# bupt-cist/vqa-playground-pytorch

Measured on AMD Instinct MI355X. Metric: VQA samples/sec (fwd+bwd), CoR2 batch 512, 36x2048 regions, higher is better.
Workload: dtype f32

## Files before the change

### vqa_playground_pytorch_amd/csrc/bilinear_rt.hip

```cpp
#include <cstdlib>

#include "bilinear_folded.hpp"
#include "gemm_f32_rt.hpp"

namespace vqa {
namespace {

struct FoldRtArgs {
  const float* x;
  const float* w[2];
  const float* bias[2];
  const float* h2;
  float* out;
  int ldx, ldw, ldh2, ldo;
  int B, N, K, NO;
  int tiles_o;
};

constexpr int kNB = 3;

template <bool FWD, int S, int IB, int R, int FG = 1>
__global__ __launch_bounds__(rt::kThreads, 1) void bilinear_fold_rt_kernel(FoldRtArgs p) {
  using rt::f32x4;
  const int lane = threadIdx.x & 63, r = lane & 15, g = lane >> 4;
  const int wave = __builtin_amdgcn_readfirstlane(threadIdx.x >> 6);
  const int tile = xcd_remap(blockIdx.x, gridDim.x);
  const int b0 = (tile / p.tiles_o) * S;
  const int o0 = (tile % p.tiles_o) * (64 * IB) + wave * (16 * IB);
  const int B = p.B, N = p.N, K = p.K, NO = p.NO;
  if (o0 >= NO) return;

  rt::rsrc_t Wb[R];
#pragma unroll
  for (int rk = 0; rk < R; ++rk) Wb[rk] = rt::make_rsrc(p.w[rk], ((size_t)(NO - 1) * p.ldw + K) * 4);
  const rt::rsrc_t Xb = rt::make_rsrc(p.x, ((size_t)(B * N - 1) * p.ldx + K) * 4);
  const rt::rsrc_t Hb = rt::make_rsrc(p.h2, (size_t)B * R * p.ldh2 * 4);
  uint32_t offW[IB], offX[S][kNB], offH[S];
#pragma unroll
  for (int i = 0; i < IB; ++i) offW[i] = ((uint32_t)min(o0 + 16 * i + r, NO - 1) * (uint32_t)p.ldw + 4u * g) * 4u;
#pragma unroll
  for (int s = 0; s < S; ++s) {
    const int b = min(b0 + s, B - 1);
#pragma unroll
    for (int j = 0; j < kNB; ++j) offX[s][j] = ((uint32_t)(b * N + min(16 * j + r, N - 1)) * (uint32_t)p.ldx + 4u * g) * 4u;
    offH[s] = (uint32_t)(b * R) * (uint32_t)p.ldh2 * 4u;
  }
  float hrow[FWD ? S : 1][R][FWD ? IB : 1];
  if constexpr (FWD) {
#pragma unroll
    for (int s = 0; s < S; ++s)
#pragma unroll
      for (int rk = 0; rk < R; ++rk)
#pragma unroll
        for (int i = 0; i < IB; ++i)
          hrow[s][rk][i] = rt::ldg4(Hb, offH[s] + (uint32_t)(rk * p.ldh2 + min(o0 + 16 * i + r, NO - 1)) * 4u, 0u);
  }

  f32x4 acc[S][IB][kNB];
#pragma unroll
  for (int s = 0; s < S; ++s)
#pragma unroll
    for (int i = 0; i < IB; ++i)
#pragma unroll
      for (int j = 0; j < kNB; ++j) acc[s][i][j] = f32x4{0.f, 0.f, 0.f, 0.f};

  struct Frag {
    f32x4 w[R][IB];
    f32x4 x[S][kNB];
    f32x4 hk[FWD ? 1 : S][R];
  };
  auto load = [&](Frag& f, int c) {
    const uint32_t so = (uint32_t)c * 64u;
#pragma unroll
    for (int rk = 0; rk < R; ++rk)
#pragma unroll
      for (int i = 0; i < IB; ++i) f.w[rk][i] = rt::ldg16(Wb[rk], offW[i], so);
#pragma unroll
    for (int s = 0; s < S; ++s) {
#pragma unroll
      for (int j = 0; j < kNB; ++j) f.x[s][j] = rt::ldg16(Xb, offX[s][j], so);
      if constexpr (!FWD) {
#pragma unroll
        for (int rk = 0; rk < R; ++rk) f.hk[s][rk] = rt::ldg16(Hb, offH[s] + (uint32_t)(rk * p.ldh2) * 4u + 16u * g, so);
      }
    }
  };
  auto fold = [&](const Frag& f, int s, int i) -> f32x4 {
    typedef float f32x2 __attribute__((ext_vector_type(2)));
    f32x4 we;
    if constexpr (FWD) {
      const f32x2 h0 = f32x2{hrow[s][0][i], hrow[s][0][i]};
      f32x2 lo = f32x2{f.w[0][i][0], f.w[0][i][1]} * h0, hi = f32x2{f.w[0][i][2], f.w[0][i][3]} * h0;
      if constexpr (R == 2) {
        const f32x2 h1 = f32x2{hrow[s][1][i], hrow[s][1][i]};
        lo = __builtin_elementwise_fma(f32x2{f.w[1][i][0], f.w[1][i][1]}, h1, lo);
        hi = __builtin_elementwise_fma(f32x2{f.w[1][i][2], f.w[1][i][3]}, h1, hi);
      }
      we = f32x4{lo[0], lo[1], hi[0], hi[1]};
    } else {
      f32x2 lo = f32x2{f.w[0][i][0], f.w[0][i][1]} * f32x2{f.hk[s][0][0], f.hk[s][0][1]};
      f32x2 hi = f32x2{f.w[0][i][2], f.w[0][i][3]} * f32x2{f.hk[s][0][2], f.hk[s][0][3]};
      if constexpr (R == 2) {
        lo = __builtin_elementwise_fma(f32x2{f.w[1][i][0], f.w[1][i][1]}, f32x2{f.hk[s][1][0], f.hk[s][1][1]}, lo);
        hi = __builtin_elementwise_fma(f32x2{f.w[1][i][2], f.w[1][i][3]}, f32x2{f.hk[s][1][2], f.hk[s][1][3]}, hi);
      }
      we = f32x4{lo[0], lo[1], hi[0], hi[1]};
    }
    return we;
  };
  auto compute = [&](const Frag& f, auto pin, auto nloads) {
    constexpr bool PIN = decltype(pin)::value;
    constexpr int NL = decltype(nloads)::value;
    constexpr int NQ = S * IB;
    constexpr int NV = R == 2 ? 4 : 2;
    f32x4 we[FG], wn[FG];
#pragma unroll
    for (int t = 0; t < FG; ++t) we[t] = fold(f, min(t, NQ - 1) / IB, min(t, NQ - 1) % IB);
    if constexpr (PIN) __builtin_amdgcn_sched_group_barrier(0x002, NV * FG, 0);
    int issued = 0;
#pragma unroll
    for (int q0 = 0; q0 < NQ; q0 += FG) {
#pragma unroll
      for (int t = 0; t < FG; ++t) wn[t] = we[t];
      if (q0 + FG < NQ) {
#pragma unroll
        for (int t = 0; t < FG; ++t)
          if (q0 + FG + t < NQ) {
            wn[t] = fold(f, (q0 + FG + t) / IB, (q0 + FG + t) % IB);
            if constexpr (PIN) __builtin_amdgcn_sched_group_barrier(0x002, NV, 0);
          }
      }
#pragma unroll
      for (int t = 0; t < FG; ++t) {
        const int q = q0 + t;
        if (q >= NQ) break;
        const int s = q / IB, i = q % IB;
#pragma unroll
        for (int kb = 0; kb < 4; ++kb)
#pragma unroll
          for (int j = 0; j < kNB; ++j) {
            acc[s][i][j] = __builtin_amdgcn_mfma_f32_16x16x4f32(we[t][kb], f.x[s][j][kb], acc[s][i][j], 0, 0, 0);
            if constexpr (PIN) {
              __builtin_amdgcn_sched_group_barrier(0x008, 1, 0);
              const int m = q * 4 * kNB + kb * kNB + j;
              if (issued < NL && (m + 1) * NL / (NQ * 4 * kNB) > issued) {
                __builtin_amdgcn_sched_group_barrier(0x020, 1, 0);
                ++issued;
              }
            }
          }
      }
#pragma unroll
      for (int t = 0; t < FG; ++t) we[t] = wn[t];
    }
  };
  auto step = [&](Frag& fn, int cn, const Frag& f) {
    constexpr int NL = R * IB + S * kNB + (FWD ? 0 : S * R);
    load(fn, cn);
    compute(f, std::true_type{}, std::integral_constant<int, NL>{});
    __builtin_amdgcn_sched_barrier(0);
  };

  const int nfull = K >> 4;
  const int c_pairs = nfull & ~1;
  {
    Frag f0, f1;
    if (c_pairs > 0) {
      load(f0, 0);
      __builtin_amdgcn_sched_barrier(0);
      for (int c = 0; c < c_pairs; c += 2) {
        step(f1, c + 1, f0);
        step(f0, min(c + 2, c_pairs - 1), f1);
      }
    }
    if (c_pairs < nfull) {
      load(f0, c_pairs);
      compute(f0, std::false_type{}, std::integral_constant<int, 0>{});
    }
  }
  if ((K & 15) != 0 || FWD) {
    Frag f;
#pragma unroll
    for (int kb = 0; kb < 4; ++kb) {
      const int k = 16 * nfull + 4 * g + kb;
      const bool in = k < K;
      const uint32_t kc = (uint32_t)min(k, K - 1);
#pragma unroll
      for (int rk = 0; rk < R; ++rk)
#pragma unroll
        for (int i = 0; i < IB; ++i) {
          float v = rt::ldg4(Wb[rk], offW[i] - 16u * g + kc * 4u, 0u);
          v = in ? v : 0.f;
          if constexpr (FWD) {
            if (k == K) v = p.bias[rk][min(o0 + 16 * i + r, NO - 1)];
          }
          f.w[rk][i][kb] = v;
        }
#pragma unroll
      for (int s = 0; s < S; ++s) {
#pragma unroll
        for (int j = 0; j < kNB; ++j) {
          float v = rt::ldg4(Xb, offX[s][j] - 16u * g + kc * 4u, 0u);
          v = in ? v : 0.f;
          if constexpr (FWD) {
            if (k == K) v = 1.f;
          }
          f.x[s][j][kb] = v;
        }
        if constexpr (!FWD) {
#pragma unroll
          for (int rk = 0; rk < R; ++rk) {
            const float v = rt::ldg4(Hb, offH[s] + (uint32_t)(rk * p.ldh2) * 4u + kc * 4u, 0u);
            f.hk[s][rk][kb] = in ? v : 0.f;
          }
        }
      }
    }
    compute(f, std::false_type{}, std::integral_constant<int, 0>{});
  }

#pragma unroll
  for (int s = 0; s < S; ++s) {
    const int b = b0 + s;
    if (b >= B) break;
#pragma unroll
    for (int j = 0; j < kNB; ++j) {
      const int n = 16 * j + r;
      if (n >= N) continue;
      float* __restrict__ row = p.out + (size_t)(b * N + n) * p.ldo;
#pragma unroll
      for (int i = 0; i < IB; ++i) {
        const int o = o0 + 16 * i + 4 * g;
        if (o + 3 < NO) {
          *reinterpret_cast<f32x4*>(row + o) = acc[s][i][j];
        } else {
#pragma unroll
          for (int t = 0; t < 4; ++t)
            if (o + t < NO) row[o + t] = acc[s][i][j][t];
        }
      }
    }
  }
}

template <bool FWD>
int launch(const FoldRtArgs& a0, int R, hipStream_t s) {
  FoldRtArgs a = a0;
  constexpr int S = FWD ? 4 : 2, IB = FWD ? 4 : 5;
  a.tiles_o = (a.NO + 64 * IB - 1) / (64 * IB);
  const dim3 grid((unsigned)(((a.B + S - 1) / S) * a.tiles_o));
  const char* fg_opt = vqa::option("VQA_K4_FG");
  const int fg = fg_opt != nullptr ? std::atoi(fg_opt) : (FWD ? 4 : 2);
  if (R == 1)
    VQA_LAUNCH((bilinear_fold_rt_kernel<FWD, S, IB, 1>), grid, dim3(rt::kThreads), 0, s, a);
  else if (fg == 2)
    VQA_LAUNCH((bilinear_fold_rt_kernel<FWD, S, IB, 2, 2>), grid, dim3(rt::kThreads), 0, s, a);
  else if (fg == 4)
    VQA_LAUNCH((bilinear_fold_rt_kernel<FWD, S, IB, 2, 4>), grid, dim3(rt::kThreads), 0, s, a);
  else
    VQA_LAUNCH((bilinear_fold_rt_kernel<FWD, S, IB, 2>), grid, dim3(rt::kThreads), 0, s, a);
  return check_launch(FWD ? "lowrank_bilinear_fusion_folded_fwd (register-tile)" : "lowrank_bilinear_fusion_folded_bwd (dx, register-tile)");
}

}

bool fold_rt_supported(int B, int N, int K, int NO, int R, int ldx, int ldw, int ldo) {
  const bool off = vqa::option_is("VQA_K4_RT", '0');
  return !off && R >= 1 && R <= 2 && N > 16 && N <= 48 && B >= 256 && K >= 32 && NO >= 64 && ldx % 2 == 0 && ldw % 2 == 0 &&
         ldo % 2 == 0 && (size_t)B * N * (size_t)(ldx > ldo ? ldx : ldo) * 4 < (1ull << 32) && (size_t)NO * ldw * 4 < (1ull << 32);
}

int fold_rt_forward(const float* x, int ldx, const float* const* w1, const float* const* b1, const float* h2, float* out, int B,
                    int N, int L, int H, int R, hipStream_t s) {
  FoldRtArgs a{};
  a.x = x;
  for (int r = 0; r < R; ++r) {
    a.w[r] = w1[r];
    a.bias[r] = b1[r];
  }
  a.h2 = h2;
  a.out = out;
  a.ldx = ldx;
  a.ldw = L;
  a.ldh2 = H;
  a.ldo = H;
  a.B = B;
  a.N = N;
  a.K = L;
  a.NO = H;
  return launch<true>(a, R, s);
}

int fold_rt_data_gradient(const float* g, const float* const* w1t, const float* h2, float* d_x, int B, int N, int L, int H, int R,
                          hipStream_t s) {
  FoldRtArgs a{};
  a.x = g;
  for (int r = 0; r < R; ++r) a.w[r] = w1t[r];
  a.h2 = h2;
  a.out = d_x;
  a.ldx = H;
  a.ldw = H;
  a.ldh2 = H;
  a.ldo = L;
  a.B = B;
  a.N = N;
  a.K = H;
  a.NO = L;
  return launch<false>(a, R, s);
}

}
```

Baseline: 262,900.

## Pack leftover regions of four samples into one shared MFMA block in fold forward

```diff
diff --git a/vqa_playground_pytorch_amd/csrc/bilinear_rt.hip b/vqa_playground_pytorch_amd/csrc/bilinear_rt.hip
--- a/vqa_playground_pytorch_amd/csrc/bilinear_rt.hip
+++ b/vqa_playground_pytorch_amd/csrc/bilinear_rt.hip
@@ -17,11 +17,11 @@
   int tiles_o;
 };
 
-constexpr int kNB = 3;
-
-template <bool FWD, int S, int IB, int R, int FG = 1>
+template <bool FWD, int S, int IB, int R, int FG = 1, int NBF = 3, bool LEFT = false>
 __global__ __launch_bounds__(rt::kThreads, 1) void bilinear_fold_rt_kernel(FoldRtArgs p) {
   using rt::f32x4;
+  static_assert(!LEFT || (FWD && S == 4), "the shared leftover block is the forward's: 4 samples x 4 regions");
+  constexpr int kNB = NBF;
   const int lane = threadIdx.x & 63, r = lane & 15, g = lane >> 4;
   const int wave = __builtin_amdgcn_readfirstlane(threadIdx.x >> 6);
   const int tile = xcd_remap(blockIdx.x, gridDim.x);
@@ -45,6 +45,9 @@
     for (int j = 0; j < kNB; ++j) offX[s][j] = ((uint32_t)(b * N + min(16 * j + r, N - 1)) * (uint32_t)p.ldx + 4u * g) * 4u;
     offH[s] = (uint32_t)(b * R) * (uint32_t)p.ldh2 * 4u;
   }
+  uint32_t offXL = 0u;
+  if constexpr (LEFT)
+    offXL = ((uint32_t)(min(b0 + (r >> 2), B - 1) * N + min(16 * NBF + (r & 3), N - 1)) * (uint32_t)p.ldx + 4u * g) * 4u;
   float hrow[FWD ? S : 1][R][FWD ? IB : 1];
   if constexpr (FWD) {
 #pragma unroll
@@ -63,10 +66,16 @@
     for (int i = 0; i < IB; ++i)
 #pragma unroll
       for (int j = 0; j < kNB; ++j) acc[s][i][j] = f32x4{0.f, 0.f, 0.f, 0.f};
+  f32x4 accL[LEFT ? R : 1][LEFT ? IB : 1];
+#pragma unroll
+  for (int rk = 0; rk < (LEFT ? R : 1); ++rk)
+#pragma unroll
+    for (int i = 0; i < (LEFT ? IB : 1); ++i) accL[rk][i] = f32x4{0.f, 0.f, 0.f, 0.f};
 
   struct Frag {
     f32x4 w[R][IB];
     f32x4 x[S][kNB];
+    f32x4 xl;
     f32x4 hk[FWD ? 1 : S][R];
   };
   auto load = [&](Frag& f, int c) {
@@ -84,6 +93,7 @@
         for (int rk = 0; rk < R; ++rk) f.hk[s][rk] = rt::ldg16(Hb, offH[s] + (uint32_t)(rk * p.ldh2) * 4u + 16u * g, so);
       }
     }
+    if constexpr (LEFT) f.xl = rt::ldg16(Xb, offXL, so);
   };
   auto fold = [&](const Frag& f, int s, int i) -> f32x4 {
     typedef float f32x2 __attribute__((ext_vector_type(2)));
@@ -113,11 +123,15 @@
     constexpr int NL = decltype(nloads)::value;
     constexpr int NQ = S * IB;
     constexpr int NV = R == 2 ? 4 : 2;
+    constexpr int NG = (NQ + FG - 1) / FG;
+    constexpr int NML = LEFT ? 4 * R * IB : 0;
+    constexpr int NM = NQ * 4 * kNB + NML;
+    static_assert(NML % NG == 0, "the shared block's MFMAs divide evenly over the fold groups");
     f32x4 we[FG], wn[FG];
 #pragma unroll
     for (int t = 0; t < FG; ++t) we[t] = fold(f, min(t, NQ - 1) / IB, min(t, NQ - 1) % IB);
     if constexpr (PIN) __builtin_amdgcn_sched_group_barrier(0x002, NV * FG, 0);
-    int issued = 0;
+    int issued = 0, m = 0;
 #pragma unroll
     for (int q0 = 0; q0 < NQ; q0 += FG) {
 #pragma unroll
@@ -130,6 +144,22 @@
             if constexpr (PIN) __builtin_amdgcn_sched_group_barrier(0x002, NV, 0);
           }
       }
+      if constexpr (LEFT) {
+#pragma unroll
+        for (int u0 = 0; u0 < NML / NG; ++u0) {
+          const int u = (q0 / FG) * (NML / NG) + u0;
+          const int kb = u / (R * IB), rk = (u / IB) % R, i = u % IB;
+          accL[rk][i] = __builtin_amdgcn_mfma_f32_16x16x4f32(f.w[rk][i][kb], f.xl[kb], accL[rk][i], 0, 0, 0);
+          if constexpr (PIN) {
+            __builtin_amdgcn_sched_group_barrier(0x008, 1, 0);
+            if (issued < NL && (m + 1) * NL / NM > issued) {
+              __builtin_amdgcn_sched_group_barrier(0x020, 1, 0);
+              ++issued;
+            }
+          }
+          ++m;
+        }
+      }
 #pragma unroll
       for (int t = 0; t < FG; ++t) {
         const int q = q0 + t;
@@ -142,12 +172,12 @@
             acc[s][i][j] = __builtin_amdgcn_mfma_f32_16x16x4f32(we[t][kb], f.x[s][j][kb], acc[s][i][j], 0, 0, 0);
             if constexpr (PIN) {
               __builtin_amdgcn_sched_group_barrier(0x008, 1, 0);
-              const int m = q * 4 * kNB + kb * kNB + j;
-              if (issued < NL && (m + 1) * NL / (NQ * 4 * kNB) > issued) {
+              if (issued < NL && (m + 1) * NL / NM > issued) {
                 __builtin_amdgcn_sched_group_barrier(0x020, 1, 0);
                 ++issued;
               }
             }
+            ++m;
           }
       }
 #pragma unroll
@@ -155,7 +185,7 @@
     }
   };
   auto step = [&](Frag& fn, int cn, const Frag& f) {
-    constexpr int NL = R * IB + S * kNB + (FWD ? 0 : S * R);
+    constexpr int NL = R * IB + S * kNB + (FWD ? 0 : S * R) + (LEFT ? 1 : 0);
     load(fn, cn);
     compute(f, std::true_type{}, std::integral_constant<int, NL>{});
     __builtin_amdgcn_sched_barrier(0);
@@ -215,6 +245,12 @@
           }
         }
       }
+      if constexpr (LEFT) {
+        float v = rt::ldg4(Xb, offXL - 16u * g + kc * 4u, 0u);
+        v = in ? v : 0.f;
+        if (k == K) v = 1.f;
+        f.xl[kb] = v;
+      }
     }
     compute(f, std::false_type{}, std::integral_constant<int, 0>{});
   }
@@ -241,6 +277,48 @@
       }
     }
   }
+  if constexpr (LEFT) {
+    const int b = b0 + (r >> 2), n = 16 * NBF + (r & 3);
+    if (b < B && n < N) {
+      float* __restrict__ row = p.out + (size_t)(b * N + n) * p.ldo;
+#pragma unroll
+      for (int i = 0; i < IB; ++i) {
+        const int o = o0 + 16 * i + 4 * g;
+        f32x4 v = f32x4{0.f, 0.f, 0.f, 0.f};
+#pragma unroll
+        for (int rk = 0; rk < R; ++rk) {
+          const uint32_t oh = (uint32_t)((b * R + rk) * p.ldh2) * 4u;
+          f32x4 h;
+          if (o + 3 < NO) {
+            h = rt::ldg16(Hb, oh + (uint32_t)o * 4u, 0u);
+          } else {
+#pragma unroll
+            for (int t = 0; t < 4; ++t) h[t] = rt::ldg4(Hb, oh + (uint32_t)min(o + t, NO - 1) * 4u, 0u);
+          }
+          v = rk == 0 ? h * accL[rk][i] : __builtin_elementwise_fma(h, accL[rk][i], v);
+        }
+        if (o + 3 < NO) {
+          *reinterpret_cast<f32x4*>(row + o) = v;
+        } else {
+#pragma unroll
+          for (int t = 0; t < 4; ++t)
+            if (o + t < NO) row[o + t] = v[t];
+        }
+      }
+    }
+  }
+}
+
+template <bool FWD, int S, int IB, int NBF, bool LEFT>
+void launch_form(const FoldRtArgs& a, int R, int fg, dim3 grid, hipStream_t s) {
+  if (R == 1)
+    VQA_LAUNCH((bilinear_fold_rt_kernel<FWD, S, IB, 1, 1, NBF, LEFT>), grid, dim3(rt::kThreads), 0, s, a);
+  else if (fg == 2)
+    VQA_LAUNCH((bilinear_fold_rt_kernel<FWD, S, IB, 2, 2, NBF, LEFT>), grid, dim3(rt::kThreads), 0, s, a);
+  else if (fg == 4)
+    VQA_LAUNCH((bilinear_fold_rt_kernel<FWD, S, IB, 2, 4, NBF, LEFT>), grid, dim3(rt::kThreads), 0, s, a);
+  else
+    VQA_LAUNCH((bilinear_fold_rt_kernel<FWD, S, IB, 2, 1, NBF, LEFT>), grid, dim3(rt::kThreads), 0, s, a);
 }
 
 template <bool FWD>
@@ -251,14 +329,12 @@
   const dim3 grid((unsigned)(((a.B + S - 1) / S) * a.tiles_o));
   const char* fg_opt = vqa::option("VQA_K4_FG");
   const int fg = fg_opt != nullptr ? std::atoi(fg_opt) : (FWD ? 4 : 2);
-  if (R == 1)
-    VQA_LAUNCH((bilinear_fold_rt_kernel<FWD, S, IB, 1>), grid, dim3(rt::kThreads), 0, s, a);
-  else if (fg == 2)
-    VQA_LAUNCH((bilinear_fold_rt_kernel<FWD, S, IB, 2, 2>), grid, dim3(rt::kThreads), 0, s, a);
-  else if (fg == 4)
-    VQA_LAUNCH((bilinear_fold_rt_kernel<FWD, S, IB, 2, 4>), grid, dim3(rt::kThreads), 0, s, a);
-  else
-    VQA_LAUNCH((bilinear_fold_rt_kernel<FWD, S, IB, 2>), grid, dim3(rt::kThreads), 0, s, a);
+  bool left = false;
+  if constexpr (FWD) left = a.N > 32 && a.N <= 36 && !vqa::option_is("VQA_K4_LEFT", '0');
+  if constexpr (FWD) {
+    if (left) launch_form<FWD, S, IB, 2, true>(a, R, fg, grid, s);
+  }
+  if (!left) launch_form<FWD, S, IB, 3, false>(a, R, fg, grid, s);
   return check_launch(FWD ? "lowrank_bilinear_fusion_folded_fwd (register-tile)" : "lowrank_bilinear_fusion_folded_bwd (dx, register-tile)");
 }
 
```

Result: no change. 262,900 (-0.0%).
